# kobanium/TamaGo

Measured on AMD Instinct MI355X. Metric: MCTS leaf-evals/sec (9x9, batch 256), higher is better.
Workload: dtype f32 results from f16 x 2 split operands, fp32 accumulate

## Files before the change

### tamago_amd/csrc/search.hip

```cpp
#include "common.h"
#define TG_RNG_DEVICE_KERNELS
#include "legacy_rng_device.h"

namespace tg {
struct LaunchCaps { int guard = 0, forward = 0; };
LaunchCaps &launch_caps();
}

#include <sched.h>

#include <cmath>
#include <cstring>
#include <algorithm>
#include <map>
#include <string>
#include <chrono>
#include <thread>
#include <condition_variable>
#include <functional>
#include <atomic>
#include <future>
#include <vector>

namespace {
// ... 590 lines not shown
            }
        } else if (i < nc) {
            double sc = pol[r] * sq;
            if (D.cgos && i == nc - 1) sc -= 0.1;
            if (best_i < 0 || sc > best) { best = sc; best_i = i; }
        }
    }
    best_i = wave_argmax_first(best, best_i);
    const int owner = best_i & 63, slot = best_i >> 6;
    int my_move = 0, my_child = 0, my_cnt = 0, my_vl = 0;
#pragma unroll
    for (int r = 0; r < R; ++r)
        if (r == slot) { my_move = act[r]; my_child = idx[r]; my_cnt = vis[r] + vl[r]; my_vl = vl[r]; }
    EdgePick pick;
    pick.edge = best_i;
    const int src = __builtin_amdgcn_readfirstlane(owner);
    pick.move = __builtin_amdgcn_readlane(my_move, src);
    pick.child = __builtin_amdgcn_readlane(my_child, src);
    pick.count = __builtin_amdgcn_readlane(my_cnt, src);
    pick.edge_vl = __builtin_amdgcn_readlane(my_vl, src);
    pick.node_vl = node_vl;
    return pick;
}

template <int S>
__device__ EdgePick select_puct(const SearchDev &D, int t, int node, int lane, const double *rcp = nullptr) {
    constexpr int A = Geo<S>::A;
    constexpr int R = (A + 63) / 64;
    const size_t ns = (size_t)t * D.N + node;
    const size_t base = ns * A;
    int vis[R], vl[R], idx[R], act[R];
    double vsum[R], pol[R];
#pragma unroll
    for (int r = 0; r < R; ++r) {
        const int i = lane + 64 * r;
        const int ii = i < A ? i : A - 1;
        vis[r] = D.ch_visits[base + ii];
        vl[r] = D.ch_vl[base + ii];
        vsum[r] = D.ch_vsum[base + ii];
        pol[r] = D.ch_policy[base + ii];
        idx[r] = D.ch_index[base + ii];
        act[r] = D.action[base + ii];
    }
    const int nc = D.node[ns].children;
    const int node_vl = D.node[ns].vl;
    const int total = D.node[ns].visits + node_vl;
    return score_puct<S>(D, vis, vl, idx, act, vsum, pol, nc, total, node_vl, lane, rcp);
}

template <int S, typename LT>
__device__ void load_root(LT &L, BoardScalars &b, int &to_move, const SearchDev &D, int t, int lane) {
    using G = Geo<S>;
    for (int p = lane; p < G::NC; p += 64) L.root_color[p] = D.root_cells[(size_t)t * G::NC + p];
    const RootMeta m = D.meta[t];
    for (int i = lane; i < m.hist_len; i += 64) L.hist[i] = D.root_hist[(size_t)t * G::HMAX + i];
    b.hash = m.hash;
    b.moves = m.moves;
    b.ko_pos = m.ko_pos;
    b.ko_move = m.ko_move;
    b.prev = m.prev;
    b.prevprev = m.prevprev;
    to_move = m.to_move;
    wave_sync();
    label_strings<S>(L.root_color, L.root_sid, lane);
}

template <int S, typename LT>
__device__ void reset_work(LT &L, int lane) {
    for (int p = lane; p < Geo<S>::NC; p += 64) { L.color[p] = L.root_color[p]; L.sid[p] = L.root_sid[p]; }
    wave_sync();
}

template <int S>
__global__ __launch_bounds__(64) void root_kernel(SearchDev D, float *planes) {
    using G = Geo<S>;
    __shared__ Lds<S> L;
    const int t = blockIdx.x, lane = threadIdx.x;
    BoardScalars b;
    int to_move;
    load_root<S>(L, b, to_move, D, t, lane);
    reset_work<S>(L, lane);
    int num_nodes = 0;
    for (int i = lane; i < G::A; i += 64) D.noise[(size_t)t * G::A + i] = 0.0;
    const int root = expand_node<S>(L, b, to_move, D, t, num_nodes, -1, -1, lane);
    write_planes<S>(L, b, to_move, planes + (size_t)t * 6 * G::P, lane);
    if (lane == 0) {
        D.meta[t].num_nodes = num_nodes;
        D.q_node[(size_t)t * D.K] = root;
        D.q_pnode[(size_t)t * D.K] = -1;
        D.q_pedge[(size_t)t * D.K] = -1;
        D.q_depth[(size_t)t * D.K] = 0;
        D.n_leaves[t] = root >= 0 ? 1 : 0;
    }
}

template <int S>
__global__ __launch_bounds__(64) void select_puct_kernel(SearchDev D, int max_leaves, float *planes) {
    using G = Geo<S>;
    constexpr int A = G::A;
    __shared__ Lds<S> L;
    const int t = blockIdx.x, lane = threadIdx.x;
    BoardScalars rootb;
    int root_to_move;
    load_root<S>(L, rootb, root_to_move, D, t, lane);
    int num_nodes = D.meta[t].num_nodes;
    int queued = 0;
    const bool prof = D.prof && t == 0;
    long long pc[8] = {0, 0, 0, 0, 0, 0, 0, 0};
    long long tp = prof ? (long long)__builtin_amdgcn_s_memtime() : 0;
    auto lap = [&](int slot) {
        if (prof) { const long long now = (long long)__builtin_amdgcn_s_memtime(); pc[slot] += now - tp; tp = now; }
    };
    if (D.err[t] == 0 && num_nodes > 0) {
        for (int k = 0; k < max_leaves; ++k) {
            reset_work<S>(L, lane);
            BoardScalars b = rootb;
            int c = root_to_move;
            int node = 0;
            bool ok = true;
            lap(0);
            for (;;) {
                const size_t ns = (size_t)t * D.N + node;
                const size_t base = ns * A;
                const EdgePick pick = select_puct<S>(D, t, node, lane);
                const int e = pick.edge;
                const int mv = pick.move;
                lap(1);
                put_stone<S>(L, b, mv, c, D.zob, lane);
                lap(2);
                if (prof) pc[7] += 1;
                c = 3 - c;
                const int edge_cnt = pick.count + 1;
                int child = pick.child;
                if (lane == 0) {
                    D.node[ns].vl = pick.node_vl + 1;
                    D.ch_vl[base + e] = pick.edge_vl + 1;
                }
                const bool two_pass = b.moves > 2 && b.prev == 0 && b.prevprev == 0;
                const int threshold = two_pass ? 10000000 : 1;
                lap(3);
                if (edge_cnt < threshold + 1) {
                    if (child == kNotExpanded) {
                        child = expand_node<S>(L, b, c, D, t, num_nodes, node, e, lane);
                        if (child < 0) { ok = false; break; }
                        if (lane == 0) D.ch_index[base + e] = child;
                    }
                    lap(4);
                    write_planes<S>(L, b, c, planes + ((size_t)t * max_leaves + k) * 6 * G::P, lane);
                    if (lane == 0) {
                        D.q_node[(size_t)t * D.K + k] = child;
                        D.q_pnode[(size_t)t * D.K + k] = node;
                        D.q_pedge[(size_t)t * D.K + k] = e;
                        D.q_depth[(size_t)t * D.K + k] = 0;
                    }
                    wave_sync();
                    lap(5);
                    break;
                }
                node = child;
                wave_sync();
                lap(3);
            }
            if (!ok) break;
            ++queued;
        }
    }
    if (lane == 0) {
        D.meta[t].num_nodes = num_nodes;
        D.n_leaves[t] = queued;
        if (prof)
            for (int i = 0; i < 8; ++i) D.prof[i] += pc[i];
    }
}

constexpr int kPipeSlots = 4;
constexpr int kPipeMaxDepth = 512;
constexpr int kPipeMaxK = 1024;
constexpr int kPipeSpinLimit = 1 << 24;

struct PipeJob {
    int k, parent, edge, child, expand, xseq, depth, src;
};

template <int S>
constexpr int kPathMax = S == 9 ? 256 : kPipeMaxDepth;

template <int S, int NW = 2>
struct PipeShared {
    static constexpr int kSlots = 2 * NW;
    Lds<S, false> board[NW];
    PipeJob job[kSlots];
    int16_t moves[kSlots][kPathMax<S>];
    int paths[kSlots][kPathMax<S>];
    int job_seq[kSlots];
    int slot_done[kSlots];
    unsigned done_bits[kPipeMaxK / 32];
    int16_t jobof[kPipeMaxK];
    int cursor_seq;
    long long cursor_val;
    int final_count;
    int err;
};

__device__ __forceinline__ int pipe_load(const int *p) {
    return __hip_atomic_load(p, __ATOMIC_ACQUIRE, __HIP_MEMORY_SCOPE_WORKGROUP);
}
__device__ __forceinline__ void pipe_store(int *p, int v) {
    __hip_atomic_store(p, v, __ATOMIC_RELEASE, __HIP_MEMORY_SCOPE_WORKGROUP);
}
template <typename Sh>
__device__ __forceinline__ void pipe_set_done(Sh &sh, int k) {
    __hip_atomic_fetch_or(&sh.done_bits[k >> 5], 1u << (k & 31), __ATOMIC_RELEASE, __HIP_MEMORY_SCOPE_WORKGROUP);
}
template <typename Sh>
__device__ __forceinline__ bool pipe_wait_done(const Sh &sh, int k);

__device__ __forceinline__ bool pipe_wait_ge(const int *p, int want) {
    for (int spin = 0; spin < kPipeSpinLimit; ++spin) {
        if (pipe_load(p) >= want) return true;
        __builtin_amdgcn_s_sleep(1);
    }
    return false;
}

template <typename Sh>
__device__ __forceinline__ bool pipe_wait_done(const Sh &sh, int k) {
    const unsigned *p = &sh.done_bits[k >> 5];
    const unsigned bit = 1u << (k & 31);
    for (int spin = 0; spin < kPipeSpinLimit; ++spin) {
        if (__hip_atomic_load(p, __ATOMIC_ACQUIRE, __HIP_MEMORY_SCOPE_WORKGROUP) & bit) return true;
        __builtin_amdgcn_s_sleep(1);
    }
    return false;
}

template <int S, typename LT>
__device__ void expand_fill(LT &L, const SearchDev &D, int t, int node, int parent, int pedge, int n, long long cur, int lane);

template <int S, typename LT, typename Sh>
__device__ bool expand_node_pipe(LT &L, const BoardScalars &b, int to_move, const SearchDev &D, int t,
                                 int node, int parent, int pedge, int xseq, Sh &sh, int lane) {
    const int n = gen_candidates<S>(L, b, to_move, D, lane);
    bool ok = pipe_wait_ge(&sh.cursor_seq, xseq);
    const long long cur = sh.cursor_val;
    if (!ok || cur + n > D.rng_cap) {
        if (lane == 0) {
            atomicOr(&D.err[t], ok ? kErrRngEmpty : kErrPipeline);
            pipe_store(&sh.err, 1);
            pipe_store(&sh.cursor_seq, xseq + 1);
        }
        return false;
    }
    if (lane == 0) {
        sh.cursor_val = cur + n;
        pipe_store(&sh.cursor_seq, xseq + 1);
    }
    expand_fill<S>(L, D, t, node, parent, pedge, n, cur, lane);
    return true;
}

template <int S, typename LT>
__device__ void expand_fill(LT &L, const SearchDev &D, int t, int node, int parent, int pedge, int n, long long cur, int lane) {
    using G = Geo<S>;
    constexpr int A = G::A;
    constexpr int R = (A + 63) / 64;
    const double *e = D.rng + (size_t)t * D.rng_cap;
    double mine[R];
#pragma unroll
    for (int r = 0; r < R; ++r) {
        long long at = cur + lane + 64 * r;
        if (at >= D.rng_cap) at = D.rng_cap - 1;
        mine[r] = e[at];
    }
    const double acc = sequential_sum<R>(mine, n);
    const double inv = 1.0 / acc;
    const size_t base = ((size_t)t * D.N + node) * A;
#pragma unroll
    for (int r = 0; r < R; ++r) {
        const int i = lane + 64 * r;
        if (i < A) {
            D.ch_index[base + i] = kNotExpanded;
            D.ch_visits[base + i] = 0;
            D.ch_vl[base + i] = 0;
            D.ch_vsum[base + i] = 0.0;
            D.ch_value[base + i] = 0.0;
            D.ch_policy[base + i] = i < n ? mine[r] * inv : 0.0;
            D.action[base + i] = i < n ? (int16_t)L.cand[i] : (int16_t)0;
        }
    }
    if (lane == 0) {
        const size_t ns = (size_t)t * D.N + node;
        D.node[ns].children = n;
        D.node[ns].visits = 0;
        D.node[ns].vl = 0;
        D.node[ns].vsum = 0.f;
        D.node[ns].raw = 0.f;
        D.node[ns].parent = parent;
        D.node[ns].pedge = pedge;
    }
    wave_sync();
}

template <int S>
__global__ __launch_bounds__(192) void select_puct_pipe_kernel(SearchDev D, int max_leaves, float *planes) {
    using G = Geo<S>;
    constexpr int A = G::A;
    __shared__ PipeShared<S> sh;
    const int t = blockIdx.x;
    const int wid = threadIdx.x >> 6, lane = threadIdx.x & 63;
    const RootMeta meta = D.meta[t];
    const int n0 = meta.num_nodes;
    if (threadIdx.x < kPipeSlots) {
        sh.job_seq[threadIdx.x] = 0;
        sh.slot_done[threadIdx.x] = 0;
    }
    for (int i = threadIdx.x; i < kPipeMaxK / 32; i += 192) sh.done_bits[i] = 0u;
    if (threadIdx.x == 0) {
        sh.cursor_seq = 0;
        sh.cursor_val = D.rng_cursor[t];
        sh.final_count = -1;
        sh.err = 0;
    }
    __syncthreads();
    const bool active = D.err[t] == 0 && n0 > 0;
    int num_nodes = n0;
    int queued = 0;

    if (wid == 0) {
        int nexp = 0;
        for (int k = 0; active && k < max_leaves; ++k) {
            if (pipe_load(&sh.err)) break;
            const int slot = k % kPipeSlots;
            bool ok = pipe_wait_ge(&sh.slot_done[slot], k / kPipeSlots);
            int node = 0, depth = 0;
            int moves = meta.moves, prev = meta.prev, prevprev = meta.prevprev;
            while (ok) {
                if (node >= n0) ok = pipe_wait_done(sh, sh.jobof[node - n0]);
                if (!ok) break;
                const size_t ns = (size_t)t * D.N + node;
                const size_t base = ns * A;
                const EdgePick pick = select_puct<S>(D, t, node, lane);
                const int e = pick.edge;
                const int mv = pick.move;
                if (depth >= kPathMax<S>) { ok = false; break; }
                if (lane == 0) {
                    sh.moves[slot][depth] = (int16_t)mv;
                    D.node[ns].vl = pick.node_vl + 1;
                    D.ch_vl[base + e] = pick.edge_vl + 1;
                    if (depth < kPathCap) D.q_path[((size_t)t * D.K + k) * kPathCap + depth] = (node << 10) | e;
                }
                ++depth;
                prevprev = prev;
                prev = mv;
                ++moves;
                const bool two_pass = moves > 2 && prev == 0 && prevprev == 0;
                const int threshold = two_pass ? 10000000 : 1;
                if (pick.count + 1 < threshold + 1) {
                    int child = pick.child;
                    const int expand = child == kNotExpanded;
                    int xseq = 0;
                    if (expand) {
                        if (num_nodes >= D.N || num_nodes - n0 >= kPipeMaxK) {
                            if (lane == 0) atomicOr(&D.err[t], kErrPoolFull);
                            ok = false;
                            break;
                        }
                        child = num_nodes++;
                        xseq = nexp++;
                    }
                    if (lane == 0) {
                        if (expand) {
                            D.ch_index[base + e] = child;
                            sh.jobof[child - n0] = (int16_t)k;
                        }
                        PipeJob &j = sh.job[slot];
                        j.k = k; j.parent = node; j.edge = e; j.child = child;
                        j.expand = expand; j.xseq = xseq; j.depth = depth;
                        D.q_node[(size_t)t * D.K + k] = child;
                        D.q_pnode[(size_t)t * D.K + k] = node;
                        D.q_pedge[(size_t)t * D.K + k] = e;
                        D.q_depth[(size_t)t * D.K + k] = (depth <= kPathCap && D.N <= (1 << 21)) ? depth : 0;
                        pipe_store(&sh.job_seq[slot], k + 1);
                    }
                    wave_sync();
                    break;
                }
                node = pick.child;
            }
            if (!ok) {
                if (lane == 0) {
                    if (!(D.err[t] & kErrPoolFull)) atomicOr(&D.err[t], kErrPipeline);
                    pipe_store(&sh.err, 1);
                }
                break;
            }
            ++queued;
        }
        if (lane == 0) pipe_store(&sh.final_count, queued);
    } else {
        Lds<S, false> &L = sh.board[wid - 1];
        BoardScalars rootb;
        int root_to_move;
        load_root<S>(L, rootb, root_to_move, D, t, lane);
        for (int k = wid - 1; active; k += 2) {
            const int slot = k % kPipeSlots;
            bool have = false, stalled = true;
            for (int spin = 0; spin < kPipeSpinLimit; ++spin) {
                if (pipe_load(&sh.job_seq[slot]) == k + 1) { have = true; stalled = false; break; }
                const int fc = pipe_load(&sh.final_count);
                if (fc >= 0 && k >= fc) { stalled = false; break; }
                __builtin_amdgcn_s_sleep(1);
            }
            if (stalled && lane == 0) {
                atomicOr(&D.err[t], kErrPipeline);
                pipe_store(&sh.err, 1);
            }
            if (!have) break;
            const PipeJob j = sh.job[slot];
            reset_work<S>(L, lane);
            BoardScalars b = rootb;
            int c = root_to_move;
            for (int i = 0; i < j.depth; ++i) {
                put_stone<S>(L, b, sh.moves[slot][i], c, D.zob, lane);
                c = 3 - c;
            }
            if (j.expand) expand_node_pipe<S>(L, b, c, D, t, j.child, j.parent, j.edge, j.xseq, sh, lane);
            write_planes<S>(L, b, c, planes + ((size_t)t * max_leaves + k) * 6 * G::P, lane);
            wave_sync();
            if (lane == 0) {
                pipe_set_done(sh, k);
                pipe_store(&sh.slot_done[slot], k / kPipeSlots + 1);
            }
        }
    }
    __syncthreads();
    if (threadIdx.x == 0) {
        D.meta[t].num_nodes = num_nodes;
        D.n_leaves[t] = queued;
        set_cursor(D, t, sh.cursor_val);
    }
}

constexpr int kMpDone = 1 << 30;
constexpr int kMpTrackDepth = 64;

template <int S, int NSEL, int NWRK>
struct MPipeShared {
    static constexpr int kMpSlots = 2 * NWRK;
    static constexpr int kRing = 2 * NSEL;
    Lds<S, false> board[NWRK];
    PipeJob job[kMpSlots];
    int16_t moves[kMpSlots][kPipeMaxDepth];
    int qpath[kMpSlots][kPathCap];
    int job_seq[kMpSlots];
    int slot_done[kMpSlots];
    int done[kPipeMaxK];
    int level_done[kPipeMaxK];
    int lvl_node[kRing][kMpTrackDepth];
    int16_t jobof[kPipeMaxK];
    int root_vl[Geo<S>::A];
    int root_idx[Geo<S>::A];
    int num_nodes, nexp;
    int cursor_seq;
    long long cursor_val;
    int err;
};

template <typename Sh>
__device__ __forceinline__ int mp_wait_val(const Sh &sh, const int *p, int want) {
    for (int spin = 0; spin < kPipeSpinLimit; ++spin) {
        const int v = pipe_load(p);
        if (v >= want) return v;
        if (spin >= 32) {
            if (pipe_load(&sh.err)) return -1;
            __builtin_amdgcn_s_sleep(1);
        }
    }
    return -1;
}
template <typename Sh>
__device__ __forceinline__ bool mp_wait_ge(const Sh &sh, const int *p, int want) {
    return mp_wait_val(sh, p, want) >= 0;
}
template <typename Sh>
__device__ __forceinline__ bool mp_wait_with(const Sh &sh, const int *flag, int want, const int *data, int &out) {
    for (int spin = 0; spin < kPipeSpinLimit; ++spin) {
        const int f = *reinterpret_cast<const volatile int *>(flag);
        const int d = *reinterpret_cast<const volatile int *>(data);
        __builtin_amdgcn_fence(__ATOMIC_ACQUIRE, "wavefront");
        if (f >= want) { out = d; return true; }
        if (spin >= 32) {
            if (pipe_load(&sh.err)) return false;
            __builtin_amdgcn_s_sleep(1);
        }
    }
    return false;
}

__device__ __forceinline__ void mp_publish(int *p, int v) {
    __builtin_amdgcn_fence(__ATOMIC_RELEASE, "wavefront");
    __hip_atomic_store(p, v, __ATOMIC_RELAXED, __HIP_MEMORY_SCOPE_WORKGROUP);
}

template <int S, int NSEL, int NWRK>
__global__ __launch_bounds__(64 * (NSEL + NWRK)) void select_puct_mpipe_kernel(SearchDev D, int max_leaves, float *planes) {
    using G = Geo<S>;
    using Shared = MPipeShared<S, NSEL, NWRK>;
    constexpr int A = G::A;
    constexpr int R = (A + 63) / 64;
    constexpr int NTHR = 64 * (NSEL + NWRK);
    constexpr int kMpSlots = Shared::kMpSlots, kRing = Shared::kRing;
    static_assert(kMpSlots % NWRK == 0 && kMpSlots >= NSEL, "job ring");
    extern __shared__ __attribute__((aligned(16))) unsigned char mp_smem[];
    Shared &sh = *reinterpret_cast<Shared *>(mp_smem);
    const int t = blockIdx.x;
    const int wid = threadIdx.x >> 6, lane = threadIdx.x & 63;
    const long long t_begin = (D.prof && t == 0) ? (long long)__builtin_amdgcn_s_memtime() : 0;
    const RootMeta meta = D.meta[t];
    const int n0 = meta.num_nodes;
    const size_t root_ns = (size_t)t * D.N, root_base = root_ns * A;
    const bool active = D.err[t] == 0 && n0 > 0;
    if (threadIdx.x < kMpSlots) {
        sh.job_seq[threadIdx.x] = 0;
        sh.slot_done[threadIdx.x] = 0;
    }
    for (int i = threadIdx.x; i < kPipeMaxK; i += NTHR) { sh.done[i] = 0; sh.level_done[i] = 0; }
    if (active)
        for (int i = threadIdx.x; i < A; i += NTHR) {
            sh.root_vl[i] = D.ch_vl[root_base + i];
            sh.root_idx[i] = D.ch_index[root_base + i];
        }
    if (threadIdx.x == 0) {
        sh.cursor_seq = 0;
        sh.cursor_val = D.rng_cursor[t];
        sh.num_nodes = n0;
        sh.nexp = 0;
        sh.err = 0;
    }
    __syncthreads();
    const bool prof = D.prof && t == 0;
    long long pc[15] = {0, 0, 0, 0, 0, 0, 0, 0, 0, 0, 0, 0, 0, 0, 0};
    long long tp = prof ? (long long)__builtin_amdgcn_s_memtime() : 0;
    auto lap = [&](int i) {
        if (prof) { const long long now = (long long)__builtin_amdgcn_s_memtime(); pc[i] += now - tp; tp = now; }
    };

    if (wid < NSEL) {
        __builtin_amdgcn_s_setprio(3);
        int r_vis[R], r_act[R], c_vl[R];
        double r_vsum[R], r_pol[R], c_q[R];
        int root_nc = 0, root_total0 = 0;
        if (active) {
#pragma unroll
            for (int r = 0; r < R; ++r) {
                const int i = lane + 64 * r, ii = i < A ? i : A - 1;
                r_vis[r] = D.ch_visits[root_base + ii];
                r_act[r] = D.action[root_base + ii];
                r_vsum[r] = D.ch_vsum[root_base + ii];
                r_pol[r] = D.ch_policy[root_base + ii];
                c_vl[r] = D.ch_vl[root_base + ii];
                const int cnt = r_vis[r] + c_vl[r];
                c_q[r] = cnt != 0 ? r_vsum[r] / (double)cnt : 0.0;
            }
            root_nc = D.node[root_ns].children;
            root_total0 = D.node[root_ns].visits + D.node[root_ns].vl;
        }
        for (int k = wid; active && k < max_leaves; k += NSEL) {
            if (pipe_load(&sh.err)) break;
            const int slot = k % kMpSlots;
            int *my_nodes = sh.lvl_node[k % kRing];
            lap(8);
            bool ok = mp_wait_ge(sh, &sh.slot_done[slot], k / kMpSlots);
            lap(0);
            int node = 0, depth = 0;
            int moves = meta.moves, prev = meta.prev;
            bool pool_full = false;
            while (ok) {
                EdgePick pick;
                size_t ns = root_ns, base = root_base;
                if (depth == 0) {
                    const double sq = __dsqrt_rn((double)(root_total0 + k + 1));
                    double psq[R], sc[R], sc1[R], q1[R];
#pragma unroll
                    for (int r = 0; r < R; ++r) {
                        const int cnt = r_vis[r] + c_vl[r];
                        psq[r] = r_pol[r] * sq;
                        sc[r] = c_q[r] + psq[r] / (double)(cnt + 1);
                        q1[r] = r_vsum[r] / (double)(cnt + 1);
                        sc1[r] = q1[r] + psq[r] / (double)(cnt + 2);
                        asm volatile("" : "+v"(sc[r]), "+v"(sc1[r]), "+v"(q1[r]), "+v"(psq[r]));
                    }
                    lap(1);
                    if (k > 0) ok = mp_wait_ge(sh, &sh.level_done[k - 1], 1);
                    lap(2);
                    if (!ok) break;
                    int idx[R];
                    bool slow = false;
                    int vl[R];
#pragma unroll
                    for (int r = 0; r < R; ++r) {
                        const int i = lane + 64 * r, ii = i < A ? i : A - 1;
                        vl[r] = sh.root_vl[ii];
                        idx[r] = sh.root_idx[ii];
                        const int d = vl[r] - c_vl[r];
                        if (d == 1) { sc[r] = sc1[r]; c_q[r] = q1[r]; c_vl[r] = vl[r]; }
                        slow |= d != 0 && d != 1;
                    }
                    if (__any(slow)) {
#pragma unroll
                        for (int r = 0; r < R; ++r)
                            if (vl[r] != c_vl[r]) {
                                c_vl[r] = vl[r];
                                const int cnt = r_vis[r] + vl[r];
                                c_q[r] = cnt != 0 ? r_vsum[r] / (double)cnt : 0.0;
                                sc[r] = c_q[r] + psq[r] / (double)(cnt + 1);
                            }
                    }
                    double best = 0.0;
                    int best_i = -1;
#pragma unroll
                    for (int r = 0; r < R; ++r) {
                        const int i = lane + 64 * r;
                        if (i < root_nc) {
                            double v = sc[r];
                            if (D.cgos && i == root_nc - 1) v -= 0.1;
                            if (best_i < 0 || v > best) { best = v; best_i = i; }
                        }
                    }
                    best_i = wave_argmax_first(best, best_i);
                    const int owner = best_i & 63, oslot = best_i >> 6;
                    int my_move = 0, my_child = 0, my_cnt = 0, my_vl = 0;
#pragma unroll
                    for (int r = 0; r < R; ++r)
                        if (r == oslot) { my_move = r_act[r]; my_child = idx[r]; my_cnt = r_vis[r] + vl[r]; my_vl = vl[r]; }
                    const int src = __builtin_amdgcn_readfirstlane(owner);
                    pick.edge = best_i;
                    pick.move = __builtin_amdgcn_readlane(my_move, src);
                    pick.child = __builtin_amdgcn_readlane(my_child, src);
                    pick.count = __builtin_amdgcn_readlane(my_cnt, src);
                    pick.edge_vl = __builtin_amdgcn_readlane(my_vl, src);
                    pick.node_vl = 0;
                    lap(3);
                } else {
                    lap(8);
                    for (int j = k - 1; ok && j > k - NSEL && j >= 0; --j) {
                        const bool tracked = depth < kMpTrackDepth;
                        const int v = mp_wait_val(sh, &sh.level_done[j], tracked ? depth : depth + 1);
                        ok = v >= 0;
                        if (ok && v == depth && sh.lvl_node[j % kRing][depth] == node)
                            ok = mp_wait_ge(sh, &sh.level_done[j], depth + 1);
                    }
                    lap(4);
                    if (ok && node >= n0) ok = mp_wait_ge(sh, &sh.done[sh.jobof[node - n0]], 1);
                    lap(5);
                    if (!ok) break;
                    ns = (size_t)t * D.N + node;
                    base = ns * A;
                    pick = select_puct<S>(D, t, node, lane);
                    lap(6);
                }
                const int e = pick.edge;
                const int mv = pick.move;
                if (depth >= kPipeMaxDepth) { ok = false; break; }
                const bool two_pass = moves + 1 > 2 && mv == 0 && prev == 0;
                const int threshold = two_pass ? 10000000 : 1;
                const bool leaf = pick.count + 1 < threshold + 1;
                if (lane == 0) {
                    if (depth == 0) {
                        sh.root_vl[e] = pick.edge_vl + 1;
                    } else {
                        D.node[ns].vl = pick.node_vl + 1;
// ... 5757 lines not shown
```

Baseline: 8.010 million.

## Cache root node edge stats in registers and raise pipe kernel occupancy for 9x9

The selector wave now loads the root node's per-edge visits, virtual loss, value sums, policy, child indices and actions into registers once per kernel, then scores the root from registers instead of re-reading global memory on every descent. It updates the cached virtual loss and child index locally as it modifies them. It also sets a min-waves-per-SIMD launch bound for the 9x9 kernel to allow more workgroups per CU, with a static_assert on LDS size. The risks are stale root visits and vsum values, since backup by other waves is not reflected in the cache, and register pressure from the double arrays under the tighter launch bound.

```diff
diff --git a/tamago_amd/csrc/search.hip b/tamago_amd/csrc/search.hip
--- a/tamago_amd/csrc/search.hip
+++ b/tamago_amd/csrc/search.hip
@@ -916,9 +916,14 @@
 }
 
 template <int S>
-__global__ __launch_bounds__(192) void select_puct_pipe_kernel(SearchDev D, int max_leaves, float *planes) {
+constexpr int kPipeWavesPerSimd = S == 9 ? 6 : 1;
+static_assert(8 * sizeof(PipeShared<9>) <= 160 * 1024, "eight select_puct_pipe_kernel<9> workgroups per CU");
+
+template <int S>
+__global__ __launch_bounds__(192, kPipeWavesPerSimd<S>) void select_puct_pipe_kernel(SearchDev D, int max_leaves, float *planes) {
     using G = Geo<S>;
     constexpr int A = G::A;
+    constexpr int R = (A + 63) / 64;
     __shared__ PipeShared<S> sh;
     const int t = blockIdx.x;
     const int wid = threadIdx.x >> 6, lane = threadIdx.x & 63;
@@ -942,6 +947,26 @@
 
     if (wid == 0) {
         int nexp = 0;
+        int r_vis[R], r_vl[R], r_idx[R], r_act[R];
+        double r_vsum[R], r_pol[R];
+        int r_nc = 0, r_visits = 0, r_node_vl = 0;
+        if (active) {
+            const size_t root_ns = (size_t)t * D.N, root_base = root_ns * A;
+#pragma unroll
+            for (int r = 0; r < R; ++r) {
+                const int i = lane + 64 * r;
+                const int ii = i < A ? i : A - 1;
+                r_vis[r] = D.ch_visits[root_base + ii];
+                r_vl[r] = D.ch_vl[root_base + ii];
+                r_vsum[r] = D.ch_vsum[root_base + ii];
+                r_pol[r] = D.ch_policy[root_base + ii];
+                r_idx[r] = D.ch_index[root_base + ii];
+                r_act[r] = D.action[root_base + ii];
+            }
+            r_nc = D.node[root_ns].children;
+            r_visits = D.node[root_ns].visits;
+            r_node_vl = D.node[root_ns].vl;
+        }
         for (int k = 0; active && k < max_leaves; ++k) {
             if (pipe_load(&sh.err)) break;
             const int slot = k % kPipeSlots;
@@ -953,7 +978,9 @@
                 if (!ok) break;
                 const size_t ns = (size_t)t * D.N + node;
                 const size_t base = ns * A;
-                const EdgePick pick = select_puct<S>(D, t, node, lane);
+                const EdgePick pick = node == 0
+                    ? score_puct<S>(D, r_vis, r_vl, r_idx, r_act, r_vsum, r_pol, r_nc, r_visits + r_node_vl, r_node_vl, lane)
+                    : select_puct<S>(D, t, node, lane);
                 const int e = pick.edge;
                 const int mv = pick.move;
                 if (depth >= kPathMax<S>) { ok = false; break; }
@@ -962,6 +989,12 @@
                     D.node[ns].vl = pick.node_vl + 1;
                     D.ch_vl[base + e] = pick.edge_vl + 1;
                     if (depth < kPathCap) D.q_path[((size_t)t * D.K + k) * kPathCap + depth] = (node << 10) | e;
+                }
+                if (node == 0) {
+                    ++r_node_vl;
+#pragma unroll
+                    for (int r = 0; r < R; ++r)
+                        if (lane + 64 * r == e) ++r_vl[r];
                 }
                 ++depth;
                 prevprev = prev;
@@ -981,6 +1014,11 @@
                         }
                         child = num_nodes++;
                         xseq = nexp++;
+                        if (node == 0) {
+#pragma unroll
+                            for (int r = 0; r < R; ++r)
+                                if (lane + 64 * r == e) r_idx[r] = child;
+                        }
                     }
                     if (lane == 0) {
                         if (expand) {
```

After: 8.094 million, median of 6. 1.01x the previous value.
